# jw0r1n/KASportsFormer

Measured on AMD Instinct MI355X. Metric: pose-clips/sec (27f x 17j) training step: fwd + 3-term loss + bwd + AdamW, higher is better.
Workload: dtype bf16; 1 GPU; SportsPose-GT 27-frame bf16 training, batch=256 per GPU (BASELINE.json configs[1]); n_layers=26, batch_per_gpu=256, global_batch=256, n_frames=27, input=ground-truth 2-D (confidence 1), 1312x1216, parallelism=single, init=reference default init, seed 114514

## Files before the change

### include/kasf.h

```cpp
#ifndef KASF_H_
#define KASF_H_
#include <stdint.h>

#ifdef __cplusplus
extern "C" {
#endif

#define KASF_DTYPE_F32 0
#define KASF_DTYPE_BF16 1

#define KASF_FLAG_TRAIN 1
#define KASF_FLAG_RETURN_REP 2
#define KASF_FLAG_KEEP 4

typedef struct kasf_model kasf_model;

typedef struct kasf_config {
    int32_t n_layers;
    int32_t n_frames;
    int32_t num_heads;
    int32_t neighbour_num;
    int32_t use_adaptive_fusion;
    int32_t dtype;
} kasf_config;
// ... 147 lines not shown
int kasf_op_attention_fwd(int32_t dtype, const void* q, int64_t ldq, const void* k, const void* v, int64_t ldkv, void* o, int32_t batch, int32_t n_frames,
                          int32_t mode, void* stream);
int kasf_op_attention_bwd(int32_t dtype, const void* q, int64_t ldq, const void* k, const void* v, int64_t ldkv, const void* d_o, void* dq, int64_t lddq,
                          void* dk, void* dv, int64_t lddkv, int32_t batch, int32_t n_frames, int32_t mode, void* stream);
int kasf_op_attention_fwd_heads(int32_t dtype, const void* q, int64_t ldq, const void* k, const void* v, int64_t ldkv, void* o, int32_t batch, int32_t n_frames,
                                int32_t mode, int32_t num_heads, void* stream);
int kasf_op_attention_bwd_heads(int32_t dtype, const void* q, int64_t ldq, const void* k, const void* v, int64_t ldkv, const void* d_o, void* dq, int64_t lddq,
                                void* dk, void* dv, int64_t lddkv, int32_t batch, int32_t n_frames, int32_t mode, int32_t num_heads, void* stream);
int kasf_op_attention_bwd_fused_do(const void* q, int64_t ldq, const void* k, const void* v, int64_t ldkv, const void* g_mid, const void* wproj_t_scaled,
                                   void* dq, int64_t lddq, void* dk, void* dv, int64_t lddkv, int32_t batch, int32_t n_frames, int32_t mode, int32_t form,
                                   const void* o_saved, const float* lse, void* stream);
#define KASF_GCN_STAT_WORDS (4 * 512 * 5)
int kasf_op_gcn_fwd(int32_t dtype, const void* x_in, const void* xn, const void* uv, const float* bn_w, const float* bn_b, float* run_mean, float* run_var,
                    const float* ls1, void* y, uint32_t* mask, void* stats, float* coef, void* out, int32_t batch, int32_t n_frames, int32_t mode,
                    int32_t neighbour_num, int32_t training, float momentum, void* stream);
int kasf_op_gcn_bwd(int32_t dtype, const void* g, const void* xn, const void* y, const float* coef, const uint32_t* mask, const float* ls1, void* r, void* duv,
                    float* dls1, float* d_bn_w, float* d_bn_b, void* bstats, int32_t batch, int32_t n_frames, int32_t mode, int32_t training, void* stream);
#define KASF_MISC_EMBED_BWD 0
#define KASF_MISC_REFUSION_BWD 1
#define KASF_MISC_GATE_BWD 2
#define KASF_MISC_HEAD_BWD 3
int64_t kasf_op_misc_scratch_floats(int32_t op, int64_t n);
int kasf_op_prologue_fwd(const kasf_model* model, const float* params, const float* x, void* xj, void* xb, void* xl, float* bone3, float* limb3, int64_t frames,
                         void* stream);
int kasf_op_embed_bwd(int32_t dtype, const void* g, const float* in3, const float* w, float* dw, float* db, float* dpos, float* din3, int64_t frames,
                      float* scratch, int64_t scratch_floats, void* stream);
int kasf_op_refusion_bwd(const kasf_model* model, const float* params, const float* x, const float* dlimb3, float* grads, int64_t frames, float* scratch,
                         int64_t scratch_floats, void* stream);
int kasf_op_gate_fwd(int32_t dtype, const void* xa, const void* xg, const void* xb, const float* w, const float* bias, void* out, float* alpha, int64_t M,
                     int32_t adaptive, void* stream);
// ... 16 lines not shown
```

### kasportsformer_amd/_lib.py

```python
from __future__ import annotations

import ctypes as C
import os

_HERE = os.path.dirname(os.path.abspath(__file__))
LIB_PATH = os.environ.get("KASF_LIB") or os.path.join(_HERE, "libkasf_hip.so")

DTYPE_F32, DTYPE_BF16 = 0, 1
DTYPE_F16 = 2
GEOM_CENTER_SCALE, GEOM_BOX = 0, 1
LAYOUT_COCO, LAYOUT_H36M = 0, 1
ROWS_PERSONS, ROWS_TRACKS = 0, 1
DETECT_PREDICTION, DETECT_HEADS = 0, 1
DETECT_MAX_CANDIDATES = 4096
LETTERBOX_MAX_SIDE = 4096
YUV_NV12, YUV_I420 = 0, 1
YUV_BT601, YUV_BT709 = 0, 1
SORT_MAX = 64
SORT_HEADER_BYTES = 64
FLAG_TRAIN, FLAG_RETURN_REP, FLAG_KEEP = 1, 2, 4
EVAL_COLS = 22
MISC_EMBED_BWD, MISC_REFUSION_BWD, MISC_GATE_BWD, MISC_HEAD_BWD = 0, 1, 2, 3
GCN_STAT_WORDS = 4 * 512 * 5
ABI_VERSION = 12
# ... 73 lines not shown
    "kasf_ws_entries": (_i32, [_vp, _i32, _i32]),
    "kasf_ws_entry": (_i32, [_vp, _i32, _i32, _i32, C.c_char_p, _i32, _pi64, _pi64, _pi32]),
    "kasf_op_linear": (_i32, [_i32, _vp, _vp, _vp, _vp, _i64, _i32, _vp, _vp, _vp, _i32, _vp]),
    "kasf_op_mlp_fwd": (_i32, [_i32, _vp, _vp, _vp, _vp, _vp, _vp, _vp, _vp, _vp, _i64, _vp, _vp]),
    "kasf_op_mlp_bwd": (_i32, [_i32, _vp, _vp, _vp, _vp, _vp, _vp, _vp, _vp, _vp, _vp, _vp, _vp, _vp, _i64, _vp]),
    "kasf_op_mlp_bwd_fused": (_i32, [_vp] * 17 + [_i64, _vp]),
    "kasf_op_wgrad": (_i32, [_i32, _vp, _i32, _vp, _i32, _vp, _vp, _vp, _vp, _i64, _vp, _i64, _vp]),
    "kasf_op_dgrad_lnbwd": (_i32, [_i32, _vp, _i32, _vp, _vp, _vp, _vp, _vp, _vp, _i32, _vp, _vp, _i64, _vp, _vp, _vp]),
    "kasf_op_attention_fwd": (_i32, [_i32, _vp, _i64, _vp, _vp, _i64, _vp, _i32, _i32, _i32, _vp]),
    "kasf_op_attention_bwd": (_i32, [_i32, _vp, _i64, _vp, _vp, _i64, _vp, _vp, _i64, _vp, _vp, _i64, _i32, _i32, _i32, _vp]),
    "kasf_op_attention_fwd_heads": (_i32, [_i32, _vp, _i64, _vp, _vp, _i64, _vp, _i32, _i32, _i32, _i32, _vp]),
    "kasf_op_attention_bwd_heads": (_i32, [_i32, _vp, _i64, _vp, _vp, _i64, _vp, _vp, _i64, _vp, _vp, _i64, _i32, _i32, _i32, _i32, _vp]),
    "kasf_op_attention_bwd_fused_do": (_i32, [_vp, _i64, _vp, _vp, _i64, _vp, _vp, _vp, _i64, _vp, _vp, _i64, _i32, _i32, _i32, _i32, _vp, _vp, _vp]),
    "kasf_op_gcn_fwd": (_i32, [_i32] + [_vp] * 13 + [_i32, _i32, _i32, _i32, _i32, _f32, _vp]),
    "kasf_op_gcn_bwd": (_i32, [_i32] + [_vp] * 12 + [_i32, _i32, _i32, _i32, _vp]),
    "kasf_op_misc_scratch_floats": (_i64, [_i32, _i64]),
    "kasf_op_prologue_fwd": (_i32, [_vp] * 8 + [_i64, _vp]),
    "kasf_op_embed_bwd": (_i32, [_i32] + [_vp] * 7 + [_i64, _vp, _i64, _vp]),
    "kasf_op_refusion_bwd": (_i32, [_vp] * 5 + [_i64, _vp, _i64, _vp]),
    "kasf_op_gate_fwd": (_i32, [_i32] + [_vp] * 7 + [_i64, _i32, _vp]),
    "kasf_op_gate_bwd": (_i32, [_i32] + [_vp] * 13 + [_i64, _i32, _vp, _i64, _vp]),
    "kasf_op_head_fwd": (_i32, [_i32] + [_vp] * 4 + [_i64, _vp]),
    "kasf_op_head_bwd": (_i32, [_i32] + [_vp] * 6 + [_i64, _vp, _i64, _vp]),
    "kasf_op_rep_bwd": (_i32, [_i32] + [_vp] * 3 + [_i64, _vp]),
    "kasf_op_finalize_ls": (_i32, [_vp] * 6 + [_i32, _i32, _vp]),
    "kasf_op_add": (_i32, [_i32] + [_vp] * 4 + [_i64, _vp]),
    "kasf_op_cast": (_i32, [_i32, _vp, _vp, _i64, _i32, _vp]),
}
_EXTRA = {}

# ... 58 lines not shown
```

### kasportsformer_amd/csrc/engine.hip

```cpp
#include <atomic>
#include <mutex>
#include <cmath>
#include <cstdio>
#include <cstring>
#include <cstdlib>
#include <string>
#include <vector>

#include "kasf.h"
#include "kernels.h"

namespace {

thread_local std::string g_err;

struct Entry { std::string name; int64_t off; int ndim; int64_t shape[4]; };

enum { KIND_ATT = 0, KIND_GRAPH = 1, KIND_BONE = 2 };
const char* const BLOCK_NAMES[6] = {"att_spatial", "att_temporal", "graph_spatial", "graph_temporal", "bone_spatial", "bone_temporal"};
const int BLOCK_KIND[6] = {KIND_ATT, KIND_ATT, KIND_GRAPH, KIND_GRAPH, KIND_BONE, KIND_BONE};
const int LIMB_N[17] = {3, 3, 2, 2, 3, 3, 4, 4, 4, 4, 3, 4, 4, 4, 4, 2, 2};

struct BlockOff {
    int kind, mode, nodes;
// ... 347 lines not shown
                                                bone ? P + o.n1lb : nullptr, c.pk(o.p_mix), bone ? c.pk(o.p_kv) : nullptr, c.pk(o.p_proj), P + o.proj_b,
                                                P + o.ls1, (c.train && w.qkv >= 0) ? c.w(w.qkv) : nullptr, (c.train && bone && w.kv >= 0) ? c.w(w.kv) : nullptr,
                                                (c.train && w.o >= 0) ? c.w(w.o) : nullptr, c.w(w.x_mid), c.B, c.T, o.mode, (c.train && w.lse >= 0) ? (float*)c.w(w.lse) : nullptr);
    }
    if (mixer_done) {
    } else if (o.kind == KIND_ATT) {
        kasf_launch_linear(c.dt, c.s, x_in, 128, c.pk(o.p_mix), 128, nullptr, c.w(w.qkv), 384, c.M, 384, P + o.n1w, P + o.n1b, nullptr, 0);
        const char* q = (const char*)c.w(w.qkv);
        kasf_launch_attn_fwd(c.dt, c.s, q, 384, q + 128 * c.es, q + 256 * c.es, 384, c.w(w.o), c.B, c.T, o.mode, heads);
    } else if (o.kind == KIND_BONE) {
        kasf_launch_linear(c.dt, c.s, x_in, 128, c.pk(o.p_mix), 128, nullptr, c.w(w.qkv), 128, c.M, 128, P + o.n1w, P + o.n1b, nullptr, 0);
        kasf_launch_linear(c.dt, c.s, x_limb, 128, c.pk(o.p_kv), 128, nullptr, c.w(w.kv), 256, c.M, 256, P + o.n1lw, P + o.n1lb, nullptr, 0);
        const char* kv = (const char*)c.w(w.kv);
        kasf_launch_attn_fwd(c.dt, c.s, c.w(w.qkv), 128, kv, kv + 128 * c.es, 256, c.w(w.o), c.B, c.T, o.mode, heads);
    } else {
        kasf_launch_linear(c.dt, c.s, x_in, 128, c.pk(o.p_mix), 128, P + o.uv_b, c.w(sc.uv), 256, c.M, 256, P + o.n1w, P + o.n1b, c.w(w.xn), 0);
        kasf_launch_gcn_agg_fwd(c.dt, c.s, c.w(sc.uv), c.w(w.xn), c.w(w.y), w.mask >= 0 ? (uint32_t*)c.w(w.mask) : nullptr, (double*)c.w(w.stats), c.B,
                                c.T, o.mode, c.m->cfg.neighbour_num);
        const double count = o.mode == 0 ? (double)c.B * c.T * 128 : (double)c.B * 17 * 128;
        kasf_launch_gcn_apply(c.dt, c.s, x_in, c.w(w.xn), c.w(w.y), (const double*)c.w(w.stats), P + o.bn_w, P + o.bn_b, c.buf + o.bn_rm, c.buf + o.bn_rv,
                              (float*)c.w(w.coef), P + o.ls1, c.w(w.x_mid), c.B, c.T, o.mode, count, c.bn_train ? 1 : 0, 0.1f);
    }
    if (o.kind != KIND_GRAPH && !mixer_done)
        kasf_launch_linear_res(c.dt, c.s, c.w(w.o), c.pk(o.p_proj), P + o.proj_b, P + o.ls1, x_in, c.w(w.x_mid), c.M);
    kasf_launch_mlp_fwd(c.dt, c.s, c.w(w.x_mid), P + o.n2w, P + o.n2b, c.pk(o.p_fc1), P + o.fc1b, c.pk(o.p_fc2), P + o.fc2b, P + o.ls2, c.w(w.x_out), c.M,
                        w.xn2 >= 0 ? c.w(w.xn2) : nullptr);
}

void block_backward(const Ctx& c, const BlockOff& o, const BlkWs& w, const void* x_in, const void* x_limb, const void* g_out, void* dst, int accumulate,
                    const Plan& p, const Scratch& sc) {
    const float* P = c.P;
    float* G = c.G;
    void* g_mid = c.w(sc.t2);
// ... 1006 lines not shown
                    int32_t neighbour_num, int32_t training, float momentum, void* stream) {
    OP_DT_CHECK(dtype);
    if (gcn_shape_check(batch, n_frames, mode) != 0) return 2;
    if (neighbour_num < 1 || neighbour_num > 4) return kasf_set_error(2, "gcn: neighbour_num must be in [1, 4]");
    if (!x_in || !xn || !uv || !bn_w || !bn_b || !run_mean || !run_var || !ls1 || !y || !stats || !coef || !out || (mode == 1 && !mask))
        return kasf_set_error(2, "null pointer argument");
    hipStream_t s = (hipStream_t)stream;
    HIPCHK(hipMemsetAsync(stats, 0, (size_t)KASF_GCN_STAT_WORDS * sizeof(int64_t), s));
    kasf_launch_gcn_agg_fwd(dtype, s, uv, xn, y, mode == 1 ? mask : nullptr, (double*)stats, batch, n_frames, mode, neighbour_num);
    const double count = mode == 0 ? (double)batch * n_frames * 128 : (double)batch * 17 * 128;
    kasf_launch_gcn_apply(dtype, s, x_in, xn, y, (const double*)stats, bn_w, bn_b, run_mean, run_var, coef, ls1, out, batch, n_frames, mode, count,
                          training ? 1 : 0, momentum);
    HIPCHK(hipGetLastError());
    return 0;
}
int kasf_op_gcn_bwd(int32_t dtype, const void* g, const void* xn, const void* y, const float* coef, const uint32_t* mask, const float* ls1, void* r, void* duv,
                    float* dls1, float* d_bn_w, float* d_bn_b, void* bstats, int32_t batch, int32_t n_frames, int32_t mode, int32_t training, void* stream) {
    OP_DT_CHECK(dtype);
    if (gcn_shape_check(batch, n_frames, mode) != 0) return 2;
    if (!g || !xn || !y || !coef || !ls1 || !r || !duv || !dls1 || !d_bn_w || !d_bn_b || !bstats || (mode == 1 && !mask))
        return kasf_set_error(2, "null pointer argument");
    hipStream_t s = (hipStream_t)stream;
    HIPCHK(hipMemsetAsync(bstats, 0, (size_t)KASF_GCN_STAT_WORDS * sizeof(int64_t), s));
    kasf_launch_gcn_bwd1(dtype, s, g, xn, y, coef, ls1, r, dls1, (double*)bstats, batch, n_frames, mode);
    const double count = mode == 0 ? (double)batch * n_frames * 128 : (double)batch * 17 * 128;
    kasf_launch_gcn_bwd2(dtype, s, r, y, coef, mode == 1 ? mask : nullptr, duv, batch, n_frames, mode, (const double*)bstats, d_bn_w, d_bn_b, count,
                         training ? 1 : 0);
    HIPCHK(hipGetLastError());
    return 0;
}
// ... 142 lines not shown
```

### kasportsformer_amd/csrc/k_gcn.hip

```cpp
#include "common.h"
#include "kernels.h"

namespace {

struct SkelTable { int nb[KASF_J][4]; float coef[KASF_J][4]; };
__constant__ SkelTable c_skel;
struct SkelLds { int nb[KASF_J][4]; __attribute__((aligned(16))) float coef[KASF_J][4]; };
__device__ __forceinline__ void skel_to_lds(SkelLds& d) {
    for (int k = threadIdx.x; k < KASF_J * 4; k += blockDim.x) {
        const int i = k >> 2, e = k & 3, nb = c_skel.nb[i][e];
        d.nb[i][e] = nb >= 0 ? nb : i;
        d.coef[i][e] = nb >= 0 ? c_skel.coef[i][e] : 0.0f;
    }
}

constexpr int COEF_LD = 8;
constexpr int MASK_W = 3;
constexpr int SX_LD = 132;

constexpr int KASF_STAT_E0 = -110;
__device__ __forceinline__ double stat_sum(const double* stats, int idx) {
    const long long* w = reinterpret_cast<const long long*>(stats);
    long long acc[KASF_STAT_WORDS];
#pragma unroll
    for (int k = 0; k < KASF_STAT_WORDS; ++k) acc[k] = 0;
#pragma unroll
    for (int sl = 0; sl < KASF_STAT_SLOTS; ++sl)
#pragma unroll
        for (int k = 0; k < KASF_STAT_WORDS; ++k) acc[k] += w[((int64_t)sl * KASF_STAT_LD + idx) * KASF_STAT_WORDS + k];
    if (acc[KASF_STAT_WORDS - 1] != 0) return __builtin_nan("");
    double v = 0.0;
#pragma unroll
    for (int k = KASF_STAT_WORDS - 2; k >= 0; --k) v += ldexp((double)acc[k], KASF_STAT_E0 + 52 * k);
    return v;
}
__device__ __forceinline__ void stat_add(double* slot, int idx, double v) {
    unsigned long long* w = reinterpret_cast<unsigned long long*>(slot) + (int64_t)idx * KASF_STAT_WORDS;
    if (v == 0.0) return;
    if (!(fabs(v) < 0x1p97)) { atomicOr(w + KASF_STAT_WORDS - 1, 1ull); return; }
    int e;
    const double m = frexp(v, &e);
    unsigned long long a = (unsigned long long)ldexp(fabs(m), 53);
    int p = e - 53 - KASF_STAT_E0;
    const bool neg = v < 0.0;
    if (p < 0) {
        const int sh = -p;
        if (sh >= 54) { a = neg ? 1 : 0; }
        else { const unsigned long long lost = a & ((1ull << sh) - 1); a >>= sh; if (neg && lost) a += 1; }
        p = 0;
        if (a == 0) return;
    }
    const int k = p / 52, r = p % 52;
    const unsigned long long lo = (a & ((1ull << (52 - r)) - 1)) << r, hi = a >> (52 - r);
    if (lo) atomicAdd(w + k, neg ? (0ull - lo) : lo);
    if (hi) atomicAdd(w + k + 1, neg ? (0ull - hi) : hi);
}
__device__ __forceinline__ double* stat_slot(double* stats) { return stats + (int64_t)(blockIdx.x % KASF_STAT_SLOTS) * KASF_STAT_LD * KASF_STAT_WORDS; }

__device__ __forceinline__ int node_of(int tok, int T, int mode) { return mode == 0 ? tok % KASF_J : (tok / KASF_J) % T; }

template <typename T>
__global__ __launch_bounds__(256) void k_gcn_agg_spatial(const T* __restrict__ uv, T* __restrict__ y, double* __restrict__ stats, int64_t M) {
    __shared__ float sStat[16][KASF_J * 2];
    __shared__ SkelLds sSk;
    for (int k = threadIdx.x; k < 16 * KASF_J * 2; k += 256) (&sStat[0][0])[k] = 0.f;
    skel_to_lds(sSk);
    __syncthreads();
    const int sub = threadIdx.x & 15, rl = threadIdx.x >> 4;
    const int n_items = (int)(M * 16);
    for (int item = blockIdx.x * 256 + threadIdx.x; item < n_items; item += gridDim.x * 256) {
        const int tk = item >> 4, fr = (tk / KASF_J) * KASF_J;
// ... 13 lines not shown
        }
        store8(y + tok * 128 + sub * 8, acc);
        float s1 = 0.f, s2 = 0.f;
#pragma unroll
        for (int k = 0; k < 8; ++k) { const float r = to_f(from_f<T>(acc[k])); s1 += r; s2 += r * r; }
        s1 = reduce16(s1);
        s2 = reduce16(s2);
        if (sub == 0) { sStat[rl][i * 2] += s1; sStat[rl][i * 2 + 1] += s2; }
    }
    __syncthreads();
    if (threadIdx.x < KASF_J * 2) {
        float t = 0.f;
#pragma unroll
        for (int k = 0; k < 16; ++k) t += sStat[k][threadIdx.x];
        stat_add(stat_slot(stats), threadIdx.x, (double)t);
    }
}

template <int L> constexpr int agg_lp() { return (L + 15) / 16 * 16; }
template <int L> constexpr int agg_ss_ld() { return (L | 1) + 1 + ((((L | 1) + 1) % 32 == 0) ? 2 : 0); }
template <typename T, int L> constexpr size_t agg_region2() {
    return (size_t)L * agg_ss_ld<L>() * sizeof(float) > (size_t)L * 128 * sizeof(T) ? (size_t)L * agg_ss_ld<L>() * sizeof(float) : (size_t)L * 128 * sizeof(T);
}
template <typename T, int L>
__global__ __launch_bounds__(256, (sizeof(T) == 2 && L == 81) ? 3 : 1) void k_gcn_agg_temporal(const T* __restrict__ uv, const T* __restrict__ xn, T* __restrict__ y,
                                                          uint32_t* __restrict__ mask, double* __restrict__ stats, int Tn, int kth, int n_tracks) {
    constexpr int LP = agg_lp<L>(), NTL = LP / 16, EPC = Tile<T>::EPC, CPR = Tile<T>::CPR, SS = agg_ss_ld<L>();
    extern __shared__ __attribute__((aligned(16))) char smem[];
    T* sX = reinterpret_cast<T*>(smem);
    T* sV = sX + LP * 128;
// ... 739 lines not shown
                                      KASF_J, count, training);
    else if (Tn == 27) bwd2_temporal_TL<T, 27>(s, r, y, coef, mask, duv, B, Tn, bstats, d_w, d_b, count, training);
    else if (Tn == 81) bwd2_temporal_TL<T, 81>(s, r, y, coef, mask, duv, B, Tn, bstats, d_w, d_b, count, training);
    else if (Tn == 9) bwd2_temporal_TL<T, 9>(s, r, y, coef, mask, duv, B, Tn, bstats, d_w, d_b, count, training);
    else {
        const int MW = kasf_gcn_mask_words(Tn);
        const size_t sh = (size_t)Tn * (128 + 16 / sizeof(T)) * sizeof(T) + (size_t)Tn * sizeof(float) + (size_t)2 * Tn * MW * sizeof(uint32_t);
        set_smem(k_gcn_bwd2_temporal_g<T>, sh);
        hipLaunchKernelGGL((k_gcn_bwd2_temporal_g<T>), dim3(B * KASF_J), dim3(256), sh, s, (const T*)r, (const T*)y, coef, mask, (T*)duv, Tn, MW, bstats, d_w,
                           d_b, count, training);
    }
}

}

void kasf_gcn_init() {
    static bool ready[64] = {};
    int dev = 0;
    (void)hipGetDevice(&dev);
    if (dev >= 0 && dev < 64 && ready[dev]) return;
    static const int adj[KASF_J][4] = {{1, 7, 4, -1}, {2, 0, -1, -1}, {3, 1, -1, -1}, {2, -1, -1, -1}, {5, 0, -1, -1}, {6, 4, -1, -1},
                                       {5, -1, -1, -1}, {0, 8, -1, -1}, {7, 9, 11, 14}, {8, 10, -1, -1}, {9, -1, -1, -1}, {12, 8, -1, -1},
                                       {13, 11, -1, -1}, {12, -1, -1, -1}, {15, 8, -1, -1}, {16, 14, -1, -1}, {15, -1, -1, -1}};
    SkelTable t;
    int deg[KASF_J];
    for (int i = 0; i < KASF_J; ++i) { deg[i] = 0; for (int e = 0; e < 4; ++e) deg[i] += adj[i][e] >= 0; }
    for (int i = 0; i < KASF_J; ++i)
        for (int e = 0; e < 4; ++e) {
            t.nb[i][e] = adj[i][e];
            t.coef[i][e] = adj[i][e] >= 0 ? (1.0f / sqrtf((float)deg[i])) * (1.0f / sqrtf((float)deg[adj[i][e]])) : 0.f;
        }
    (void)hipMemcpyToSymbol(HIP_SYMBOL(c_skel), &t, sizeof(t));
    if (dev >= 0 && dev < 64) ready[dev] = true;
}

void kasf_launch_gcn_agg_fwd(int dt, hipStream_t s, const void* uv, const void* xn, void* y, uint32_t* mask, double* stats, int B, int T, int mode, int kth) {
    kasf_gcn_init();
    if (dt == KASF_F32) agg_fwd_T<float>(s, uv, xn, y, mask, stats, B, T, mode, kth);
    else agg_fwd_T<bf16>(s, uv, xn, y, mask, stats, B, T, mode, kth);
}
void kasf_launch_gcn_apply(int dt, hipStream_t s, const void* x_in, const void* xn, const void* y, const double* stats, const float* bn_w, const float* bn_b,
                           float* run_mean, float* run_var, float* coef, const float* ls1, void* out, int B, int T, int mode, double count, int training,
                           float momentum) {
    const int64_t M = (int64_t)B * T * KASF_J;
    const int nodes = mode == 0 ? KASF_J : T;
    if (dt == KASF_F32) hipLaunchKernelGGL(k_gcn_apply<float>, dim3(ew_grid(M)), dim3(256), 0, s, (const float*)x_in, (const float*)xn, (const float*)y, stats, bn_w, bn_b, run_mean, run_var, coef, ls1, (float*)out, M, T, mode, nodes, count, training, momentum);
    else hipLaunchKernelGGL(k_gcn_apply<bf16>, dim3(ew_grid(M)), dim3(256), 0, s, (const bf16*)x_in, (const bf16*)xn, (const bf16*)y, stats, bn_w, bn_b, run_mean, run_var, coef, ls1, (bf16*)out, M, T, mode, nodes, count, training, momentum);
}
// ... 19 lines not shown
```

### kasportsformer_amd/csrc/k_gemm2.hip

```cpp
#include "common.h"
#include "kernels.h"
#include "tile_ops.h"
#include "mlp_fin.h"
#ifndef KASF_LINEAR_ISSUE_AT
#define KASF_LINEAR_ISSUE_AT 1
#endif

namespace {

constexpr int R_BM = 32, R_NW = 8, R_THR = R_NW * 64;
constexpr int R_TILE = R_BM * 128;

__device__ __forceinline__ f32x4 mfma16(bf16x8 a, bf16x8 b, f32x4 c) { return __builtin_amdgcn_mfma_f32_16x16x32_bf16(a, b, c, 0, 0, 0); }
__device__ __forceinline__ bf16x8 tok_frag(const bf16* s, int row, int ks) {
    const int g = (threadIdx.x & 63) >> 4;
    return *reinterpret_cast<const bf16x8*>(s + Tile<bf16>::chunk_off(row, 4 * ks + g));
}

template <int KC, bool RESID, bool ADD, bool ACC, bool XN, int RING, bool WG = false, bool BIAS = false, bool PROJ = false, bool MLPFIN = false>
__global__ __launch_bounds__(R_THR) void k_dgrad_r(const bf16* __restrict__ dY, const bf16* __restrict__ Wt, const bf16* __restrict__ dxn_add,
                                                   const bf16* __restrict__ X, const float* __restrict__ gamma, const float* __restrict__ beta,
                                                   const bf16* __restrict__ resid, bf16* __restrict__ out, float* __restrict__ dgamma,
                                                   float* __restrict__ dbeta, bf16* __restrict__ xn_out, int64_t M, float* __restrict__ part,
                                                   bf16* __restrict__ wpart, float* __restrict__ dbias, const bf16* __restrict__ Oin,
// ... 436 lines not shown
}

template <int NC, bool LN, bool RES>
void launch_linear_r(hipStream_t s, const void* A, const void* W, const float* bias, const float* ln_g, const float* ln_b, void* xn_out, const float* ls,
                     const void* resid, void* C, int64_t M) {
    const size_t sh = (size_t)(3 * (1 + (RES ? 1 : 0)) + (LN ? 2 : 0) + NC) * R_TILE * 2;
    auto kern = k_linear_r<NC, LN, RES>;
    (void)hipFuncSetAttribute(reinterpret_cast<const void*>(kern), hipFuncAttributeMaxDynamicSharedMemorySize, (int)sh);
    const int64_t tiles = (M + R_BM - 1) / R_BM;
    const int64_t gcap = kasf_narrow_grid(KASF_NG_LINEAR, 256, M);
    const unsigned grid = (unsigned)(tiles < gcap ? tiles : gcap);
    hipLaunchKernelGGL(kern, dim3(grid), dim3(R_THR), sh, s, (const bf16*)A, (const bf16*)W, bias, ln_g, ln_b, (bf16*)xn_out, ls, (const bf16*)resid,
                       (bf16*)C, M);
}

}

bool kasf_launch_dgrad_r(hipStream_t s, const void* dY, int Kd, const void* Wt, const void* dxn_add, const void* X, const float* gamma, const void* resid,
                         void* out, int accumulate, float* dgamma, float* dbeta, int64_t M, void* xn_out, const float* beta, KasfColSink* sink) {
    const bool R = resid != nullptr, A = dxn_add != nullptr, C = accumulate != 0, XN = xn_out != nullptr;
    if (M <= 0) return true;
    if (Kd == 384 && R && !A && !C && XN) launch_dgrad_r<3, true, false, false, true>(s, dY, Wt, dxn_add, X, gamma, beta, resid, out, dgamma, dbeta, xn_out, M, sink);
    else if (Kd == 128 && R && !A && !C && XN) launch_dgrad_r<1, true, false, false, true>(s, dY, Wt, dxn_add, X, gamma, beta, resid, out, dgamma, dbeta, xn_out, M, sink);
    else if (Kd == 256 && !R && !A && C && XN) launch_dgrad_r<2, false, false, true, true>(s, dY, Wt, dxn_add, X, gamma, beta, resid, out, dgamma, dbeta, xn_out, M, sink);
    else if (Kd == 256 && R && A && !C && !XN) launch_dgrad_r<2, true, true, false, false>(s, dY, Wt, dxn_add, X, gamma, beta, resid, out, dgamma, dbeta, xn_out, M, sink);
    else return false;
    return true;
}

bool kasf_dgrad_wg_supported(int Kd, bool resid, bool accumulate, bool dxn_add, bool dbias, bool proj, int64_t M, int64_t wpart_bytes) {
// ... 39 lines not shown
    const int grid = (int)(tiles < gcap ? tiles : gcap);
    const int64_t per = (tiles + grid - 1) / grid;
    const int active = (int)((tiles + per - 1) / per);
    float* part = sink != nullptr ? sink->take(active, PLD) : nullptr;
    hipLaunchKernelGGL(kern, dim3(grid + 128), dim3(R_THR), sh, s, (const bf16*)dZ, (const bf16*)W1t, (const bf16*)nullptr, (const bf16*)X, gamma, (const float*)nullptr,
                       (const bf16*)g, (bf16*)g_in, dgamma, dbeta, (bf16*)nullptr, M, part, (bf16*)nullptr, gsum, (const bf16*)nullptr, (bf16*)nullptr,
                       (float*)nullptr, *reinterpret_cast<const MlpFinArgs*>(fin_args), grid);
    if (part != nullptr) {
        sink->add(part, PLD, active, 128, dgamma);
        sink->add(part + 128, PLD, active, 128, dbeta);
        if (have_w2) sink->add(part + 256, PLD, active, 128, gsum, 1, b2, ls2, dls2);
        else sink->add(part + 256, PLD, active, 128, gsum);
    }
}

bool kasf_launch_linear_r(hipStream_t s, const void* A, const void* W, const float* bias, void* C, int64_t M, int N, const float* ln_g, const float* ln_b,
                          void* xn_out) {
    if (M <= 0) return true;
    const bool ln = ln_g != nullptr;
    if (N == 384 && ln) launch_linear_r<3, true, false>(s, A, W, bias, ln_g, ln_b, xn_out, nullptr, nullptr, C, M);
    else if (N == 256 && ln) launch_linear_r<2, true, false>(s, A, W, bias, ln_g, ln_b, xn_out, nullptr, nullptr, C, M);
    else if (N == 128 && ln) launch_linear_r<1, true, false>(s, A, W, bias, ln_g, ln_b, xn_out, nullptr, nullptr, C, M);
    else if (N == 128 && !ln && xn_out == nullptr) launch_linear_r<1, false, false>(s, A, W, bias, nullptr, nullptr, nullptr, nullptr, nullptr, C, M);
    else return false;
    return true;
}
void kasf_launch_linear_res_r(hipStream_t s, const void* A, const void* W, const float* bias, const float* ls, const void* resid, void* C, int64_t M) {
    if (M <= 0) return;
    launch_linear_r<1, false, true>(s, A, W, bias, nullptr, nullptr, nullptr, ls, resid, C, M);
}
// ... 1 lines not shown
```

### kasportsformer_amd/csrc/kernels.h

```cpp
#pragma once
#include <hip/hip_runtime.h>
#include <stdint.h>

#define KASF_F32 0
#define KASF_BF16 1
#define KASF_F16 2

struct KasfPackDesc {
    int64_t src;
    int64_t dst;
    int64_t scale;
    int rows, cols;
    int transpose;
    int fp16;
};

struct KasfProOff {
    int64_t mlp[51][4];
    int64_t embed_w[3];
    int64_t embed_b[3];
    int64_t pos[3];
};

int kasf_set_error(int code, const char* msg);
// ... 54 lines not shown

void kasf_launch_attn_fwd(int dt, hipStream_t s, const void* q, int64_t ldq, const void* k, const void* v, int64_t ldkv, void* o, int B, int T,
                          int mode, int heads = 8);
void kasf_launch_attn_bwd(int dt, hipStream_t s, const void* q, int64_t ldq, const void* k, const void* v, int64_t ldkv, const void* d_o, void* dq,
                          int64_t lddq, void* dk, void* dv, int64_t lddkv, int B, int T, int mode, int heads = 8);

bool kasf_launch_attn_fwd_mfma(hipStream_t s, const void* q, int64_t ldq, const void* k, const void* v, int64_t ldkv, void* o, int B, int T, int mode);
bool kasf_launch_attn_bwd_mfma(hipStream_t s, const void* q, int64_t ldq, const void* k, const void* v, int64_t ldkv, const void* d_o, void* dq,
                               int64_t lddq, void* dk, void* dv, int64_t lddkv, int B, int T, int mode);
bool kasf_launch_attn_fwd_mfma32(hipStream_t s, const void* q, int64_t ldq, const void* k, const void* v, int64_t ldkv, void* o, int B, int T, int mode);
bool kasf_launch_attn_bwd_mfma32(hipStream_t s, const void* q, int64_t ldq, const void* k, const void* v, int64_t ldkv, const void* d_o, void* dq, int64_t lddq,
                                 void* dk, void* dv, int64_t lddkv, int B, int T, int mode);

void kasf_gcn_init();
void kasf_launch_gcn_agg_fwd(int dt, hipStream_t s, const void* uv, const void* xn, void* y, uint32_t* mask, double* stats, int B, int T, int mode, int kth = 4);
void kasf_launch_gcn_apply(int dt, hipStream_t s, const void* x_in, const void* xn, const void* y, const double* stats, const float* bn_w, const float* bn_b,
                           float* run_mean, float* run_var, float* coef, const float* ls1, void* out, int B, int T, int mode, double count, int training,
                           float momentum);
void kasf_launch_gcn_bwd1(int dt, hipStream_t s, const void* g, const void* xn, const void* y, const float* coef, const float* ls1, void* r,
                          float* dls1, double* bstats, int B, int T, int mode, KasfColSink* sink = nullptr);
void kasf_launch_gcn_bwd2(int dt, hipStream_t s, const void* r, const void* y, const float* coef, const uint32_t* mask, void* duv, int B, int T,
                          int mode, const double* bstats, float* d_bn_w, float* d_bn_b, double count, int training = 1);

int64_t kasf_misc_scratch_floats(int op, int64_t n, int refusion_len);
void kasf_launch_prologue_fwd(int dt, hipStream_t s, const float* x, const float* params, const KasfProOff* off, void* xj, void* xb, void* xl,
                              float* bone3, float* limb3, int64_t frames);
void kasf_launch_embed_bwd(int dt, hipStream_t s, const void* g, const float* in3, const float* W, float* dW, float* db, float* dpos, float* din3,
                           int64_t frames, KasfColSink* sink = nullptr);
void kasf_launch_refusion_bwd(hipStream_t s, const float* x, const float* dlimb3, const float* params, float* grads, const KasfProOff* off,
                              int64_t frames, KasfColSink* sink = nullptr, int64_t grad_base = 0, int grad_len = 0);
// ... 143 lines not shown
```

Baseline: 4725 pose-clips/sec.

## Fuse GCN LayerNorm, uv projection and spatial aggregation into one kernel

```diff
diff --git a/include/kasf.h b/include/kasf.h
--- a/include/kasf.h
+++ b/include/kasf.h
@@ -185,6 +185,9 @@
 int kasf_op_gcn_fwd(int32_t dtype, const void* x_in, const void* xn, const void* uv, const float* bn_w, const float* bn_b, float* run_mean, float* run_var,
                     const float* ls1, void* y, uint32_t* mask, void* stats, float* coef, void* out, int32_t batch, int32_t n_frames, int32_t mode,
                     int32_t neighbour_num, int32_t training, float momentum, void* stream);
+#define KASF_GCN_NO_FUSED_FORM 7
+int kasf_op_gcn_mix_fwd(int32_t dtype, const void* x, const float* ln_g, const float* ln_b, const void* w_uv, const float* b_uv, void* xn_out, void* y_out,
+                        uint32_t* mask_out, void* stats_out, int32_t batch, int32_t n_frames, int32_t mode, int32_t neighbour_num, void* stream);
 int kasf_op_gcn_bwd(int32_t dtype, const void* g, const void* xn, const void* y, const float* coef, const uint32_t* mask, const float* ls1, void* r, void* duv,
                     float* dls1, float* d_bn_w, float* d_bn_b, void* bstats, int32_t batch, int32_t n_frames, int32_t mode, int32_t training, void* stream);
 #define KASF_MISC_EMBED_BWD 0
diff --git a/kasportsformer_amd/_lib.py b/kasportsformer_amd/_lib.py
--- a/kasportsformer_amd/_lib.py
+++ b/kasportsformer_amd/_lib.py
@@ -111,6 +111,7 @@
     "kasf_op_attention_bwd_fused_do": (_i32, [_vp, _i64, _vp, _vp, _i64, _vp, _vp, _vp, _i64, _vp, _vp, _i64, _i32, _i32, _i32, _i32, _vp, _vp, _vp]),
     "kasf_op_gcn_fwd": (_i32, [_i32] + [_vp] * 13 + [_i32, _i32, _i32, _i32, _i32, _f32, _vp]),
     "kasf_op_gcn_bwd": (_i32, [_i32] + [_vp] * 12 + [_i32, _i32, _i32, _i32, _vp]),
+    "kasf_op_gcn_mix_fwd": (_i32, [_i32] + [_vp] * 9 + [_i32, _i32, _i32, _i32, _vp]),
     "kasf_op_misc_scratch_floats": (_i64, [_i32, _i64]),
     "kasf_op_prologue_fwd": (_i32, [_vp] * 8 + [_i64, _vp]),
     "kasf_op_embed_bwd": (_i32, [_i32] + [_vp] * 7 + [_i64, _vp, _i64, _vp]),
diff --git a/kasportsformer_amd/csrc/engine.hip b/kasportsformer_amd/csrc/engine.hip
--- a/kasportsformer_amd/csrc/engine.hip
+++ b/kasportsformer_amd/csrc/engine.hip
@@ -385,9 +385,16 @@
         const char* kv = (const char*)c.w(w.kv);
         kasf_launch_attn_fwd(c.dt, c.s, c.w(w.qkv), 128, kv, kv + 128 * c.es, 256, c.w(w.o), c.B, c.T, o.mode, heads);
     } else {
-        kasf_launch_linear(c.dt, c.s, x_in, 128, c.pk(o.p_mix), 128, P + o.uv_b, c.w(sc.uv), 256, c.M, 256, P + o.n1w, P + o.n1b, c.w(w.xn), 0);
-        kasf_launch_gcn_agg_fwd(c.dt, c.s, c.w(sc.uv), c.w(w.xn), c.w(w.y), w.mask >= 0 ? (uint32_t*)c.w(w.mask) : nullptr, (double*)c.w(w.stats), c.B,
-                                c.T, o.mode, c.m->cfg.neighbour_num);
+        const char* fe = getenv("KASF_GCN_FUSED_FWD");
+        const bool fused = c.dt == KASF_BF16 && !(fe != nullptr && fe[0] == '0') &&
+                           kasf_launch_gcn_mix_fwd(c.dt, c.s, x_in, P + o.n1w, P + o.n1b, c.pk(o.p_mix), P + o.uv_b, c.w(w.xn), c.w(w.y),
+                                                   w.mask >= 0 ? (uint32_t*)c.w(w.mask) : nullptr, (double*)c.w(w.stats), c.w(sc.uv), (int64_t)c.M * 256 * c.es, c.B,
+                                                   c.T, o.mode, c.m->cfg.neighbour_num);
+        if (!fused) {
+            kasf_launch_linear(c.dt, c.s, x_in, 128, c.pk(o.p_mix), 128, P + o.uv_b, c.w(sc.uv), 256, c.M, 256, P + o.n1w, P + o.n1b, c.w(w.xn), 0);
+            kasf_launch_gcn_agg_fwd(c.dt, c.s, c.w(sc.uv), c.w(w.xn), c.w(w.y), w.mask >= 0 ? (uint32_t*)c.w(w.mask) : nullptr, (double*)c.w(w.stats), c.B,
+                                    c.T, o.mode, c.m->cfg.neighbour_num);
+        }
         const double count = o.mode == 0 ? (double)c.B * c.T * 128 : (double)c.B * 17 * 128;
         kasf_launch_gcn_apply(c.dt, c.s, x_in, c.w(w.xn), c.w(w.y), (const double*)c.w(w.stats), P + o.bn_w, P + o.bn_b, c.buf + o.bn_rm, c.buf + o.bn_rv,
                               (float*)c.w(w.coef), P + o.ls1, c.w(w.x_mid), c.B, c.T, o.mode, count, c.bn_train ? 1 : 0, 0.1f);
@@ -1424,6 +1431,30 @@
     HIPCHK(hipGetLastError());
     return 0;
 }
+int kasf_op_gcn_mix_fwd(int32_t dtype, const void* x, const float* ln_g, const float* ln_b, const void* w_uv, const float* b_uv, void* xn_out, void* y_out,
+                        uint32_t* mask_out, void* stats_out, int32_t batch, int32_t n_frames, int32_t mode, int32_t neighbour_num, void* stream) {
+    OP_DT_CHECK(dtype);
+    if (gcn_shape_check(batch, n_frames, mode) != 0) return 2;
+    if (neighbour_num < 1 || neighbour_num > 4) return kasf_set_error(2, "gcn: neighbour_num must be in [1, 4]");
+    if (!x || !ln_g || !ln_b || !w_uv || !b_uv || !xn_out || !y_out || !stats_out || (mode == 1 && !mask_out)) return kasf_set_error(2, "null pointer argument");
+    if (!kasf_gcn_mix_fwd_supported(dtype, n_frames, mode))
+        return kasf_set_error(KASF_GCN_NO_FUSED_FORM, "gcn_mix_fwd: no fused form for this dtype / mode / n_frames (bf16 spatial only): run kasf_op_linear + kasf_op_gcn_fwd");
+    hipStream_t s = (hipStream_t)stream;
+    const int64_t M = (int64_t)batch * n_frames * 17;
+    void* tokstat = nullptr;
+    HIPCHK(hipMallocAsync(&tokstat, (size_t)M * 8, s));
+    hipError_t e = hipMemsetAsync(stats_out, 0, (size_t)KASF_GCN_STAT_WORDS * sizeof(int64_t), s);
+    bool ok = false;
+    if (e == hipSuccess) {
+        ok = kasf_launch_gcn_mix_fwd(dtype, s, x, ln_g, ln_b, w_uv, b_uv, xn_out, y_out, mode == 1 ? mask_out : nullptr, (double*)stats_out, tokstat, M * 8, batch, n_frames,
+                                     mode, neighbour_num);
+        e = hipGetLastError();
+    }
+    (void)hipFreeAsync(tokstat, s);
+    HIPCHK(e);
+    if (!ok) return kasf_set_error(KASF_GCN_NO_FUSED_FORM, "gcn_mix_fwd: no fused form for this shape");
+    return 0;
+}
 int kasf_op_gcn_bwd(int32_t dtype, const void* g, const void* xn, const void* y, const float* coef, const uint32_t* mask, const float* ls1, void* r, void* duv,
                     float* dls1, float* d_bn_w, float* d_bn_b, void* bstats, int32_t batch, int32_t n_frames, int32_t mode, int32_t training, void* stream) {
     OP_DT_CHECK(dtype);
diff --git a/kasportsformer_amd/csrc/k_gcn.hip b/kasportsformer_amd/csrc/k_gcn.hip
--- a/kasportsformer_amd/csrc/k_gcn.hip
+++ b/kasportsformer_amd/csrc/k_gcn.hip
@@ -34,8 +34,7 @@
     for (int k = KASF_STAT_WORDS - 2; k >= 0; --k) v += ldexp((double)acc[k], KASF_STAT_E0 + 52 * k);
     return v;
 }
-__device__ __forceinline__ void stat_add(double* slot, int idx, double v) {
-    unsigned long long* w = reinterpret_cast<unsigned long long*>(slot) + (int64_t)idx * KASF_STAT_WORDS;
+__device__ __forceinline__ void stat_add_words(unsigned long long* w, double v) {
     if (v == 0.0) return;
     if (!(fabs(v) < 0x1p97)) { atomicOr(w + KASF_STAT_WORDS - 1, 1ull); return; }
     int e;
@@ -55,6 +54,9 @@
     if (lo) atomicAdd(w + k, neg ? (0ull - lo) : lo);
     if (hi) atomicAdd(w + k + 1, neg ? (0ull - hi) : hi);
 }
+__device__ __forceinline__ void stat_add(double* slot, int idx, double v) {
+    stat_add_words(reinterpret_cast<unsigned long long*>(slot) + (int64_t)idx * KASF_STAT_WORDS, v);
+}
 __device__ __forceinline__ double* stat_slot(double* stats) { return stats + (int64_t)(blockIdx.x % KASF_STAT_SLOTS) * KASF_STAT_LD * KASF_STAT_WORDS; }
 
 __device__ __forceinline__ int node_of(int tok, int T, int mode) { return mode == 0 ? tok % KASF_J : (tok / KASF_J) % T; }
@@ -98,6 +100,48 @@
 #pragma unroll
         for (int k = 0; k < 16; ++k) t += sStat[k][threadIdx.x];
         stat_add(stat_slot(stats), threadIdx.x, (double)t);
+    }
+}
+
+constexpr int REPLAY_VW = 16;
+__global__ __launch_bounds__(256) void k_gcn_stat_replay(const float2* __restrict__ tokstat, double* __restrict__ stats, int64_t M, int vgrid) {
+    __shared__ float sStat[256][KASF_J * 2 + 1];
+    __shared__ unsigned long long sAcc[KASF_STAT_SLOTS * KASF_J * 2 * KASF_STAT_WORDS];
+    for (int k = threadIdx.x; k < 256 * (KASF_J * 2 + 1); k += 256) (&sStat[0][0])[k] = 0.f;
+    for (int k = threadIdx.x; k < KASF_STAT_SLOTS * KASF_J * 2 * KASF_STAT_WORDS; k += 256) sAcc[k] = 0ull;
+    __syncthreads();
+    const int n_tok = (int)M, step = vgrid * 16;
+    {
+        const int vb = (int)blockIdx.x * REPLAY_VW + (threadIdx.x >> 4), rl = threadIdx.x & 15;
+        if (vb < vgrid) {
+#pragma unroll 4
+            for (int tk = vb * 16 + rl; tk < n_tok; tk += step) {
+                const float2 v = tokstat[tk];
+                const int i = tk % KASF_J;
+                sStat[threadIdx.x][i * 2] += v.x;
+                sStat[threadIdx.x][i * 2 + 1] += v.y;
+            }
+        }
+    }
+    __syncthreads();
+    for (int idx = threadIdx.x; idx < REPLAY_VW * KASF_J * 2; idx += 256) {
+        const int v = idx / (KASF_J * 2), c = idx - v * (KASF_J * 2), vb = (int)blockIdx.x * REPLAY_VW + v;
+        if (vb < vgrid) {
+            float t = 0.f;
+#pragma unroll
+            for (int k = 0; k < 16; ++k) t += sStat[v * 16 + k][c];
+            stat_add_words(sAcc + ((vb % KASF_STAT_SLOTS) * KASF_J * 2 + c) * KASF_STAT_WORDS, (double)t);
+        }
+    }
+    __syncthreads();
+    unsigned long long* w = reinterpret_cast<unsigned long long*>(stats);
+    for (int idx = threadIdx.x; idx < KASF_STAT_SLOTS * KASF_J * 2 * KASF_STAT_WORDS; idx += 256) {
+        const unsigned long long a = sAcc[idx];
+        if (a == 0ull) continue;
+        const int sl = idx / (KASF_J * 2 * KASF_STAT_WORDS), rem = idx - sl * (KASF_J * 2 * KASF_STAT_WORDS), c = rem / KASF_STAT_WORDS, k = rem - c * KASF_STAT_WORDS;
+        unsigned long long* dst = w + ((int64_t)sl * KASF_STAT_LD + c) * KASF_STAT_WORDS + k;
+        if (k == KASF_STAT_WORDS - 1) atomicOr(dst, a);
+        else atomicAdd(dst, a);
     }
 }
 
@@ -867,15 +911,10 @@
 
 }
 
-void kasf_gcn_init() {
-    static bool ready[64] = {};
-    int dev = 0;
-    (void)hipGetDevice(&dev);
-    if (dev >= 0 && dev < 64 && ready[dev]) return;
+static void skel_table(SkelTable& t) {
     static const int adj[KASF_J][4] = {{1, 7, 4, -1}, {2, 0, -1, -1}, {3, 1, -1, -1}, {2, -1, -1, -1}, {5, 0, -1, -1}, {6, 4, -1, -1},
                                        {5, -1, -1, -1}, {0, 8, -1, -1}, {7, 9, 11, 14}, {8, 10, -1, -1}, {9, -1, -1, -1}, {12, 8, -1, -1},
                                        {13, 11, -1, -1}, {12, -1, -1, -1}, {15, 8, -1, -1}, {16, 14, -1, -1}, {15, -1, -1, -1}};
-    SkelTable t;
     int deg[KASF_J];
     for (int i = 0; i < KASF_J; ++i) { deg[i] = 0; for (int e = 0; e < 4; ++e) deg[i] += adj[i][e] >= 0; }
     for (int i = 0; i < KASF_J; ++i)
@@ -883,8 +922,30 @@
             t.nb[i][e] = adj[i][e];
             t.coef[i][e] = adj[i][e] >= 0 ? (1.0f / sqrtf((float)deg[i])) * (1.0f / sqrtf((float)deg[adj[i][e]])) : 0.f;
         }
+}
+void kasf_gcn_init() {
+    static bool ready[64] = {};
+    int dev = 0;
+    (void)hipGetDevice(&dev);
+    if (dev >= 0 && dev < 64 && ready[dev]) return;
+    SkelTable t;
+    skel_table(t);
     (void)hipMemcpyToSymbol(HIP_SYMBOL(c_skel), &t, sizeof(t));
     if (dev >= 0 && dev < 64) ready[dev] = true;
+}
+void kasf_gcn_skel_arg(KasfSkelArg* out) {
+    SkelTable t;
+    skel_table(t);
+    for (int i = 0; i < KASF_J; ++i)
+        for (int e = 0; e < 4; ++e) {
+            out->nb[i][e] = t.nb[i][e] >= 0 ? t.nb[i][e] : i;
+            out->coef[i][e] = t.nb[i][e] >= 0 ? t.coef[i][e] : 0.0f;
+        }
+}
+void kasf_launch_gcn_stat_replay(hipStream_t s, const float* tokstat, double* stats, int64_t M) {
+    unsigned grid = ew_grid(M);
+    if (grid > 1024) grid = 1024;
+    hipLaunchKernelGGL(k_gcn_stat_replay, dim3((grid + REPLAY_VW - 1) / REPLAY_VW), dim3(256), 0, s, reinterpret_cast<const float2*>(tokstat), stats, M, (int)grid);
 }
 
 void kasf_launch_gcn_agg_fwd(int dt, hipStream_t s, const void* uv, const void* xn, void* y, uint32_t* mask, double* stats, int B, int T, int mode, int kth) {
diff --git a/kasportsformer_amd/csrc/k_gemm2.hip b/kasportsformer_amd/csrc/k_gemm2.hip
--- a/kasportsformer_amd/csrc/k_gemm2.hip
+++ b/kasportsformer_amd/csrc/k_gemm2.hip
@@ -474,6 +474,170 @@
                        (bf16*)C, M);
 }
 
+
+template <int FR>
+__global__ __launch_bounds__(R_THR) void k_gcn_mix_spatial(const bf16* __restrict__ X, const bf16* __restrict__ W, const float* __restrict__ bias,
+                                                           const float* __restrict__ ln_g, const float* __restrict__ ln_b, bf16* __restrict__ xn_out,
+                                                           bf16* __restrict__ Y, float2* __restrict__ tokstat, const KasfSkelArg skel, int64_t M) {
+    constexpr int ROWS = FR * KASF_J, NI = (ROWS + 3) / 4, IPW = (NI + R_NW - 1) / R_NW, SLOT = NI * 4 * 128;
+    constexpr int MT = (ROWS + 15) / 16, PT = MT * 16 * 128, NP = (ROWS + 31) / 32;
+    static_assert((IPW - 1) * R_NW < NI, "every wave's last request is a real instruction or the shared last one");
+    extern __shared__ __attribute__((aligned(16))) char smem[];
+    __shared__ KasfSkelArg sSk;
+    bf16* sRing = reinterpret_cast<bf16*>(smem);
+    bf16* sA = sRing + 3 * SLOT;
+    bf16* sO = sA + PT;
+    const int w = threadIdx.x >> 6, lane = threadIdx.x & 63, i = lane & 15, g = lane >> 4, sub = lane & 15, rl = threadIdx.x >> 4;
+    const int64_t ntiles_total = (M + ROWS - 1) / ROWS;
+    const int64_t per = (ntiles_total + gridDim.x - 1) / gridDim.x;
+    const int64_t tile0 = (int64_t)blockIdx.x * per;
+    int64_t ntiles = ntiles_total - tile0;
+    if (ntiles > per) ntiles = per;
+    if (ntiles <= 0) return;
+    for (int k = threadIdx.x; k < KASF_J * 4; k += R_THR) { sSk.nb[k >> 2][k & 3] = skel.nb[k >> 2][k & 3]; sSk.coef[k >> 2][k & 3] = skel.coef[k >> 2][k & 3]; }
+
+    bf16x8 wf[2][4];
+    f32x4 bv[2];
+#pragma unroll
+    for (int nt = 0; nt < 2; ++nt) {
+#pragma unroll
+        for (int ks = 0; ks < 4; ++ks) wf[nt][ks] = *reinterpret_cast<const bf16x8*>(W + (int64_t)(32 * w + 16 * nt + i) * 128 + 32 * ks + 8 * g);
+        bv[nt] = *reinterpret_cast<const f32x4*>(bias + 32 * w + 16 * nt + 4 * g);
+    }
+    float gm[8], bt[8];
+#pragma unroll
+    for (int e = 0; e < 8; ++e) { gm[e] = ln_g[sub * 8 + e]; bt[e] = ln_b[sub * 8 + e]; }
+    __syncthreads();
+#pragma unroll
+    for (int nt = 0; nt < 2; ++nt) {
+        touch_loaded(bv[nt]);
+#pragma unroll
+        for (int ks = 0; ks < 4; ++ks) touch_loaded(wf[nt][ks]);
+    }
+
+    auto nx3 = [](int sl) { return sl == 2 ? 0 : sl + 1; };
+    const int wu = __builtin_amdgcn_readfirstlane(w);
+    auto issue = [&](int64_t t, int sl) {
+        const int64_t tt = t < ntiles ? t : ntiles - 1;
+        const int64_t row0 = (tile0 + tt) * ROWS;
+        const int nvalid = (int)((M - row0) < ROWS ? (M - row0) : ROWS);
+        const unsigned base = __builtin_amdgcn_readfirstlane(lds_addr(sRing + sl * SLOT));
+        const void* ub = uniform_ptr(X + row0 * 128);
+#pragma unroll
+        for (int q = 0; q < IPW; ++q) {
+            const int inst = wu + R_NW * q < NI - 1 ? wu + R_NW * q : NI - 1;
+            const int row = inst * 4 + (lane >> 4), c = (lane & 15) ^ (row & 15);
+            const int srow = row < nvalid ? row : nvalid - 1;
+            glds16_s(ub, (unsigned)srow * 256u + (unsigned)c * 16u, base + (unsigned)inst * 1024u);
+        }
+    };
+    auto layernorm = [&](int64_t t, int sl) {
+#pragma unroll
+        for (int p = 0; p < NP; ++p) {
+            const int r = 32 * p + rl;
+            if (32 * (p + 1) <= ROWS || r < ROWS) {
+                float v[8];
+                tile_load8(sRing + sl * SLOT, r, sub * 8, v);
+                float s = 0.f;
+#pragma unroll
+                for (int e = 0; e < 8; ++e) s += v[e];
+                const float mean = reduce16(s) * (1.0f / 128.0f);
+                float q = 0.f;
+#pragma unroll
+                for (int e = 0; e < 8; ++e) { v[e] -= mean; q += v[e] * v[e]; }
+                const float rstd = rsqrtf(reduce16(q) * (1.0f / 128.0f) + KASF_LN_EPS);
+#pragma unroll
+                for (int e = 0; e < 8; ++e) v[e] = v[e] * rstd * gm[e] + bt[e];
+                tile_store8(sA, r, sub * 8, v);
+                const int64_t row = (tile0 + t) * ROWS + r;
+                if (row < M) store8(xn_out + row * 128 + sub * 8, v);
+            }
+        }
+    };
+    issue(0, 0);
+    issue(1, 1);
+    wait_async_le<IPW>();
+    layernorm(0, 0);
+    int sl = 0;
+    for (int64_t t = 0; t < ntiles; ++t, sl = nx3(sl)) {
+        const int64_t row0 = (tile0 + t) * ROWS;
+        barrier_keep_async();
+        issue(t + 2, nx3(nx3(sl)));
+        {
+            f32x4 acc[2][MT];
+            zero_acc(acc);
+#pragma unroll
+            for (int ks = 0; ks < 4; ++ks) {
+#pragma unroll
+                for (int mt = 0; mt < MT; ++mt) {
+                    const bf16x8 fb = tok_frag(sA, mt * 16 + i, ks);
+                    acc[0][mt] = mfma16(wf[0][ks], fb, acc[0][mt]);
+                    acc[1][mt] = mfma16(wf[1][ks], fb, acc[1][mt]);
+                }
+            }
+#pragma unroll
+            for (int nt = 0; nt < 2; ++nt)
+#pragma unroll
+                for (int mt = 0; mt < MT; ++mt) {
+                    const int col = 32 * w + 16 * nt + 4 * g;
+                    float v[4];
+#pragma unroll
+                    for (int r = 0; r < 4; ++r) v[r] = acc[nt][mt][r] + bv[nt][r];
+                    store4(sO + (col >> 7) * PT + Tile<bf16>::off4(mt * 16 + i, col & 127), v);
+                }
+        }
+        barrier_keep_async();
+        wait_async_le<IPW>();
+        if (t + 1 < ntiles) layernorm(t + 1, nx3(sl));
+#pragma unroll
+        for (int p = 0; p < NP; ++p) {
+            const int r = 32 * (p + 1) <= ROWS ? 32 * p + rl : 32 * p + rl - (32 - (ROWS - 32 * p));
+            const int64_t tok = row0 + r;
+            const bool full = 32 * (p + 1) <= ROWS;
+            if (full || r >= 32 * p) {
+                const int fr = (r / KASF_J) * KASF_J, jn = r - fr;
+                const f32x4 cf = *reinterpret_cast<const f32x4*>(sSk.coef[jn]);
+                const int nbs[4] = {sSk.nb[jn][0], sSk.nb[jn][1], sSk.nb[jn][2], sSk.nb[jn][3]};
+                float acc[8], v[4][8];
+                tile_load8(sO, r, sub * 8, acc);
+#pragma unroll
+                for (int e = 0; e < 4; ++e) tile_load8(sO + PT, fr + nbs[e], sub * 8, v[e]);
+#pragma unroll
+                for (int e = 0; e < 4; ++e) {
+                    const float c = cf[e];
+#pragma unroll
+                    for (int k = 0; k < 8; ++k) acc[k] += c * v[e][k];
+                }
+                float s1 = 0.f, s2 = 0.f;
+#pragma unroll
+                for (int k = 0; k < 8; ++k) { const float rr = (float)(bf16)acc[k]; s1 += rr; s2 += rr * rr; }
+                s1 = reduce16(s1);
+                s2 = reduce16(s2);
+                if (tok < M) {
+                    store8(Y + tok * 128 + sub * 8, acc);
+                    if (sub == 0) tokstat[tok] = make_float2(s1, s2);
+                }
+            }
+        }
+    }
+    wait_async();
+}
+
+template <int FR>
+void launch_gcn_mix_spatial(hipStream_t s, const void* X, const void* W, const float* bias, const float* ln_g, const float* ln_b, void* xn_out, void* Y, void* tokstat,
+                            int64_t M) {
+    constexpr int ROWS = FR * KASF_J, NI = (ROWS + 3) / 4, MT = (ROWS + 15) / 16;
+    const size_t sh = (size_t)(3 * NI * 4 + 3 * MT * 16) * 128 * 2;
+    auto kern = k_gcn_mix_spatial<FR>;
+    (void)hipFuncSetAttribute(reinterpret_cast<const void*>(kern), hipFuncAttributeMaxDynamicSharedMemorySize, (int)sh);
+    KasfSkelArg skel;
+    kasf_gcn_skel_arg(&skel);
+    const int64_t tiles = (M + ROWS - 1) / ROWS;
+    const int64_t gcap = kasf_narrow_grid(KASF_NG_LINEAR, 256, M);
+    const unsigned grid = (unsigned)(tiles < gcap ? tiles : gcap);
+    hipLaunchKernelGGL(kern, dim3(grid), dim3(R_THR), sh, s, (const bf16*)X, (const bf16*)W, bias, ln_g, ln_b, (bf16*)xn_out, (bf16*)Y, (float2*)tokstat, skel, M);
+}
+
 }
 
 bool kasf_launch_dgrad_r(hipStream_t s, const void* dY, int Kd, const void* Wt, const void* dxn_add, const void* X, const float* gamma, const void* resid,
@@ -543,6 +707,19 @@
     }
 }
 
+#ifndef KASF_GCN_MIX_FR
+#define KASF_GCN_MIX_FR 4
+#endif
+bool kasf_gcn_mix_fwd_supported(int dt, int T, int mode) { return dt == KASF_BF16 && mode == 0 && T >= 1; }
+bool kasf_launch_gcn_mix_fwd(int dt, hipStream_t s, const void* x, const float* ln_g, const float* ln_b, const void* w_uv, const float* b_uv, void* xn, void* y,
+                             uint32_t* mask, double* stats, void* scratch, int64_t scratch_bytes, int B, int T, int mode, int kth) {
+    (void)mask; (void)kth;
+    const int64_t M = (int64_t)B * T * KASF_J;
+    if (!kasf_gcn_mix_fwd_supported(dt, T, mode) || M <= 0 || scratch == nullptr || scratch_bytes < M * 8) return false;
+    launch_gcn_mix_spatial<KASF_GCN_MIX_FR>(s, x, w_uv, b_uv, ln_g, ln_b, xn, y, scratch, M);
+    kasf_launch_gcn_stat_replay(s, (const float*)scratch, stats, M);
+    return true;
+}
 bool kasf_launch_linear_r(hipStream_t s, const void* A, const void* W, const float* bias, void* C, int64_t M, int N, const float* ln_g, const float* ln_b,
                           void* xn_out) {
     if (M <= 0) return true;
diff --git a/kasportsformer_amd/csrc/kernels.h b/kasportsformer_amd/csrc/kernels.h
--- a/kasportsformer_amd/csrc/kernels.h
+++ b/kasportsformer_amd/csrc/kernels.h
@@ -92,6 +92,12 @@
 
 void kasf_gcn_init();
 void kasf_launch_gcn_agg_fwd(int dt, hipStream_t s, const void* uv, const void* xn, void* y, uint32_t* mask, double* stats, int B, int T, int mode, int kth = 4);
+struct KasfSkelArg { int nb[17][4]; float coef[17][4]; };
+void kasf_gcn_skel_arg(KasfSkelArg* out);
+void kasf_launch_gcn_stat_replay(hipStream_t s, const float* tokstat, double* stats, int64_t M);
+bool kasf_gcn_mix_fwd_supported(int dt, int T, int mode);
+bool kasf_launch_gcn_mix_fwd(int dt, hipStream_t s, const void* x, const float* ln_g, const float* ln_b, const void* w_uv, const float* b_uv, void* xn, void* y,
+                             uint32_t* mask, double* stats, void* scratch, int64_t scratch_bytes, int B, int T, int mode, int kth);
 void kasf_launch_gcn_apply(int dt, hipStream_t s, const void* x_in, const void* xn, const void* y, const double* stats, const float* bn_w, const float* bn_b,
                            float* run_mean, float* run_var, float* coef, const float* ls1, void* out, int B, int T, int mode, double count, int training,
                            float momentum);
```

Result: slower. 4669 pose-clips/sec (-1.2%).
